# baowj-678/koordinator

Hardware: AMD Instinct MI355X
Metric: pods placed/sec + (pod,node) Filter+Score evals/sec at 50k nodes, 1-8 GPUs (higher is better)
Workload: dtype int64; 1 GPU; config4: 50000 nodes x 100000 pods, 30% BE, NodeResourcesFit + LoadAwareScheduling, shipped scheduler-config.yaml profile; nodes=50000, pods=100000, batch_pods=24, pipeline_lag=2, parallelism=node-shard x1

## Files before the change

koordinator_amd/csrc/eval.hpp:

```cpp
#pragma once
#include <hip/hip_runtime.h>
#include <stdint.h>

#include "../../include/koordhip.h"
#include "numa.hpp"

namespace kh {

template <typename T>
__device__ __forceinline__ void st_wt(T *p, T v) {
  if constexpr (sizeof(T) == 8) {
    __hip_atomic_store(reinterpret_cast<uint64_t *>(p), __builtin_bit_cast(uint64_t, v), __ATOMIC_RELAXED,
                       __HIP_MEMORY_SCOPE_AGENT);
  } else if constexpr (sizeof(T) == 4) {
    __hip_atomic_store(reinterpret_cast<uint32_t *>(p), __builtin_bit_cast(uint32_t, v), __ATOMIC_RELAXED,
                       __HIP_MEMORY_SCOPE_AGENT);
  } else {
    __hip_atomic_store(reinterpret_cast<uint8_t *>(p), __builtin_bit_cast(uint8_t, v), __ATOMIC_RELAXED,
                       __HIP_MEMORY_SCOPE_AGENT);
  }
}

enum : uint32_t {
  NF_LA_OK_NONPROD = 1u,
  NF_LA_OK_PROD = 2u,
  NF_LA_SCORE_ZERO = 4u,
  NF_OVER_CPU = 8u,
  NF_OVER_MEM = 16u,
  NF_OVER_EPH = 32u,
};

struct DevCfg {
  uint32_t filt, score;
  int32_t w_fit, w_la, w_numa, w_bal;
  int32_t fit_w[KOORDHIP_NRES];
  int32_t la_w_cpu, la_w_mem;
  int32_t according;
  int32_t la_alias;
  int32_t numa_w_cpu, numa_w_mem;
  int32_t numa_most;
  int32_t zones;
  int32_t amp;
  int32_t resv;
  int32_t resv_slots;
  int32_t resv_cpus;
  int32_t resv_b1;
  int32_t wide_keys;
  int32_t w_ext[KOORDHIP_NEXT_PLUGINS];
  int32_t dev_most;
  int32_t dev_w[5];
};

struct DevDev {
  int32_t slots;
  const uint8_t *present;
  const int32_t *minor;
  const int64_t *total;
  int64_t *used;
  const int64_t *xalloc;
  int64_t *xreq;
  const uint16_t *sscore[2];
  const int32_t *rslot;
  int64_t *rdev;
  const int64_t *rxa;
  int64_t *rxd;
};

struct DevNodes {
  const double *alloc[KOORDHIP_NRES];
  const int32_t *alloc_pods;
  double *requested[KOORDHIP_NRES];
  double *nz_cpu, *nz_mem;
// ... 68 lines not shown
  if (ns) {
    n.r_cpu |= !is_cpuset(p);
    n.r_mem = true;
    n.a_cpu = n.a_mem = true;
  }
  if (c.score & KOORDHIP_PLUGIN_BALANCED) n.r_cpu = n.r_mem = n.a_cpu = n.a_mem = true;
  n.sa = (c.filt & KOORDHIP_PLUGIN_NODE_STATIC) != 0;
  if (c.resv) {
    n.resv = true;
    n.r_cpu = n.r_mem = n.pods = true;
    n.eph |= (c.filt & KOORDHIP_PLUGIN_RESERVATION) && p.resv_match != 0ull;
  }
  n.a_cpu = n.a_cpu || n.r_cpu || n.nz_cpu || (n.la && c.la_alias);
  n.a_mem = n.a_mem || n.r_mem || n.nz_mem || (n.la && c.la_alias);
  return n;
}

__device__ __forceinline__ void need_or(Need &a, const Need &b) {
  a.pods |= b.pods;
  a.r_cpu |= b.r_cpu;
  a.r_mem |= b.r_mem;
  a.eph |= b.eph;
  a.bcpu |= b.bcpu;
  a.bmem |= b.bmem;
  a.a_cpu |= b.a_cpu;
  a.a_mem |= b.a_mem;
  a.nz_cpu |= b.nz_cpu;
  a.nz_mem |= b.nz_mem;
  a.la |= b.la;
  a.la_nonprod |= b.la_nonprod;
  a.la_prod |= b.la_prod;
  a.numa |= b.numa;
  a.numa_masks |= b.numa_masks;
  a.zones |= b.zones;
  a.amp |= b.amp;
  a.resv |= b.resv;
}

__device__ __forceinline__ Need need_all(const DevCfg &c) {
  Need n{};
  n.pods = n.r_cpu = n.r_mem = n.eph = n.bcpu = n.bmem = n.a_cpu = n.a_mem = n.nz_cpu = n.nz_mem = true;
  n.la = true;
  n.la_nonprod = true;
  n.la_prod = c.according != 0;
  n.numa = n.numa_masks = numa_on(c);
  n.zones = n.numa && c.zones;
  n.amp = n.numa && c.amp;
  n.resv = c.resv != 0;
  n.sa = true;
  return n;
}

__device__ __forceinline__ void load_zones(NumaRow &r, const DevNodes &d, int32_t i) {
  const double *zu = d.nu.zu + (size_t)i * 2 * ZMAX;
  r.za = d.nu.za + (size_t)i * 2 * ZMAX;
#pragma unroll
  for (int q = 0; q < ZMAX; q++) {
    r.zu[0][q] = zu[q];
    r.zu[1][q] = zu[ZMAX + q];
  }
}

template <bool Z>
__device__ __forceinline__ void load_numa(NumaRow &r, const DevNodes &d, int32_t i, const Need &n) {
  r.cls = -1;
  r.nflags = 0;
  r.amp = 1.0;
  if (!n.numa) return;
  r.cls = d.nu.node_cls[i];
  if (n.amp) {
    r.amp = d.nu.amp[i];
    r.cnt = d.nu.cnt[i];
  }
  if (n.numa_masks || (Z && n.zones)) r.nflags = d.nu.nflags[i];
  if constexpr (Z) {
    if (n.zones && topo_policy(r.nflags) != 0) load_zones(r, d, i);
  }
  if (n.numa_masks) {
    r.cnt = d.nu.cnt[i];
#pragma unroll
    for (int w = 0; w < NW; w++) {
      r.fr[w] = d.nu.fr[w][i];
      r.ep[w] = d.nu.ep[w][i];
      r.en[w] = d.nu.en[w][i];
    }
  }
}

template <typename T>
__device__ __forceinline__ const T &col(const T *base, int32_t i) {
  return *reinterpret_cast<const T *>(reinterpret_cast<const char *>(base) + (uint32_t)i * (uint32_t)sizeof(T));
}
template <typename T>
__device__ __forceinline__ T &col(T *base, int32_t i) {
  return *reinterpret_cast<T *>(reinterpret_cast<char *>(base) + (uint32_t)i * (uint32_t)sizeof(T));
}

__device__ __forceinline__ void load_node(NV &v, const DevNodes &d, int32_t i, const Need &n, const DevCfg &c) {
  v.flags = col(d.flags, i);
  v.sa = (n.sa && d.sallow) ? col(d.sallow, i) : 0xFFFFFFFFu;
  if (n.pods) {
    v.a_pods = col(d.alloc_pods, i);
    v.npods = col(d.npods, i);
  }
  if (n.a_cpu) v.a[KOORDHIP_RES_CPU] = col(d.alloc[KOORDHIP_RES_CPU], i);
  if (n.a_mem) v.a[KOORDHIP_RES_MEM] = col(d.alloc[KOORDHIP_RES_MEM], i);
  if (n.r_cpu) v.r[KOORDHIP_RES_CPU] = col(d.requested[KOORDHIP_RES_CPU], i);
// ... 266 lines not shown
    resv_pref_cpus(r, p, (c.score & KOORDHIP_PLUGIN_RESERVATION) ? mm : 0u, P, rx);
    NumaRow q = r;
    if (topo_policy(q.nflags) != 0) load_zones(q, *zd, zi);
    t = eval_total_numa<true>(p, w, q, classes, c, P);
  } else if constexpr (RC && S > 1) {
    uint64_t P[NW];
    resv_pref_cpus(r, p, (c.score & KOORDHIP_PLUGIN_RESERVATION) ? mm : 0u, P, rx);
    t = eval_total_numa<false>(p, w, r, classes, c, P);
  } else {
    t = eval_total_numa<false>(p, w, r, classes, c);
  }
  if (t < 0) return t;
  if (nmatch == 0)
    return ((c.filt & KOORDHIP_PLUGIN_RESERVATION) && (p.flags & KOORDHIP_POD_RESV_AFFINITY)) ? -1 : t;
  if ((c.filt & KOORDHIP_PLUGIN_RESERVATION) && !resv_filter(p, w, r, mm, nmatch, rx)) return -1;
  if (c.score & KOORDHIP_PLUGIN_RESERVATION) {
    const int rk = resv_node_rank(r, mm);
    if (rk >= 0) return 101 * c.resv_b1 + (KOORDHIP_RESV_MAX_ORDERS - 1 - rk);
    const int q = resv_nominate(p, r, mm, rx);
    if (q >= 0) t += resv_score(p, r.rs[q], q == rx.h, rx) * c.resv_b1;
  }
  return t;
}

__device__ __forceinline__ uint64_t make_key(int32_t total, int32_t node) {
  return total < 0 ? 0ull : (((uint64_t)(uint32_t)(total + 1)) << 32) | (uint64_t)(0xFFFFFFFFu - (uint32_t)node);
}
__device__ __forceinline__ int32_t key_node(uint64_t k) { return (int32_t)(0xFFFFFFFFu - (uint32_t)k); }
__device__ __forceinline__ int32_t key_score(uint64_t k) { return (int32_t)(k >> 32) - 1; }

__device__ __forceinline__ void apply_delta(NV &v, const DevPod &p, int sign) {
  const double sg = (double)sign;
#pragma unroll
  for (int r = 0; r < KOORDHIP_NRES; r++) v.r[r] = __builtin_fma(sg, p.req[r], v.r[r]);
  v.nz_cpu = __builtin_fma(sg, p.nz_cpu_m, v.nz_cpu);
  v.nz_mem = __builtin_fma(sg, p.nz_mem, v.nz_mem);
  v.npods += sign;
  v.la_u_cpu = __builtin_fma(sg, p.est_cpu, v.la_u_cpu);
  v.la_u_mem = __builtin_fma(sg, p.est_mem, v.la_u_mem);
  if (p.flags & KOORDHIP_POD_PROD) {
    v.la_up_cpu = __builtin_fma(sg, p.est_cpu, v.la_up_cpu);
    v.la_up_mem = __builtin_fma(sg, p.est_mem, v.la_up_mem);
  }
  uint32_t f = v.flags & ~(NF_OVER_CPU | NF_OVER_MEM | NF_OVER_EPH);
  if (v.r[KOORDHIP_RES_CPU] > v.a[KOORDHIP_RES_CPU]) f |= NF_OVER_CPU;
  if (v.r[KOORDHIP_RES_MEM] > v.a[KOORDHIP_RES_MEM]) f |= NF_OVER_MEM;
  if (v.r[KOORDHIP_RES_EPH] > v.a[KOORDHIP_RES_EPH]) f |= NF_OVER_EPH;
  v.flags = f;
}

__device__ __forceinline__ void load_row(NV &v, const DevNodes &d, int32_t i) {
#pragma unroll
  for (int r = 0; r < KOORDHIP_NRES; r++) {
    v.a[r] = d.alloc[r][i];
    v.r[r] = d.requested[r][i];
  }
  v.a_pods = d.alloc_pods[i];
  v.npods = d.npods[i];
  v.nz_cpu = d.nz_cpu[i];
  v.nz_mem = d.nz_mem[i];
  v.la_a_cpu = d.la_alloc_cpu[i];
  v.la_a_mem = d.la_alloc_mem[i];
  v.la_u_cpu = d.la_used_cpu[i];
  v.la_u_mem = d.la_used_mem[i];
  v.la_up_cpu = d.la_used_prod_cpu[i];
  v.la_up_mem = d.la_used_prod_mem[i];
  v.flags = d.flags[i];
  v.sa = d.sallow ? d.sallow[i] : 0xFFFFFFFFu;
}

template <bool Z = true>
__device__ __forceinline__ void load_numa_row(NumaRow &r, const DevNodes &d, int32_t i) {
  r.cls = d.nu.node_cls[i];
  r.nflags = d.nu.nflags[i];
  r.cnt = d.nu.cnt[i];
#pragma unroll
  for (int w = 0; w < NW; w++) {
    r.fr[w] = d.nu.fr[w][i];
    r.ep[w] = d.nu.ep[w][i];
    r.en[w] = d.nu.en[w][i];
  }
  if (Z && d.nu.za && topo_policy(r.nflags) != 0) load_zones(r, d, i);
  r.amp = d.nu.amp ? d.nu.amp[i] : 1.0;
}

template <bool Z = true>
__device__ __forceinline__ void store_numa_row(const NumaRow &r, const DevNodes &d, int32_t i) {
  d.nu.cnt[i] = r.cnt;
#pragma unroll
  for (int w = 0; w < NW; w++) {
    d.nu.fr[w][i] = r.fr[w];
    d.nu.ep[w][i] = r.ep[w];
    d.nu.en[w][i] = r.en[w];
  }
  if (Z && d.nu.za && topo_policy(r.nflags) != 0) {
    double *zu = d.nu.zu + (size_t)i * 2 * ZMAX;
#pragma unroll
    for (int q = 0; q < ZMAX; q++) {
      zu[q] = r.zu[0][q];
      zu[ZMAX + q] = r.zu[1][q];
    }
  }
}

__device__ __forceinline__ void numa_apply(NumaRow &r, const DevPod &p, const uint64_t *cpus, int sign,
                                           const uint64_t *P = nullptr) {
  const int ex = (int)KOORDHIP_NUMA_EXCLUSIVE(p.numa_policy);
  int n = 0;
#pragma unroll
  for (int w = 0; w < NW; w++) {
    n += __popcll(P ? (cpus[w] & ~P[w]) : cpus[w]);
    if (sign > 0) {
      r.fr[w] &= ~cpus[w];
      r.ep[w] = (r.ep[w] & ~cpus[w]) | (ex == (int)KOORDHIP_CPUEXCL_PCPU ? cpus[w] : 0ull);
      r.en[w] = (r.en[w] & ~cpus[w]) | (ex == (int)KOORDHIP_CPUEXCL_NUMA ? cpus[w] : 0ull);
    } else {
      r.fr[w] |= cpus[w];
      r.ep[w] &= ~cpus[w];
      r.en[w] &= ~cpus[w];
    }
  }
  r.cnt += sign * n;
}

__device__ __forceinline__ void store_row(const NV &v, const DevNodes &d, int32_t i) {
#pragma unroll
  for (int r = 0; r < KOORDHIP_NRES; r++) d.requested[r][i] = v.r[r];
  d.npods[i] = v.npods;
  d.nz_cpu[i] = v.nz_cpu;
  d.nz_mem[i] = v.nz_mem;
  d.la_used_cpu[i] = v.la_u_cpu;
  d.la_used_mem[i] = v.la_u_mem;
  d.la_used_prod_cpu[i] = v.la_up_cpu;
  d.la_used_prod_mem[i] = v.la_up_mem;
  d.flags[i] = (uint8_t)v.flags;
}

__device__ __forceinline__ void store_row_wt(const NV &v, const DevNodes &d, int32_t i) {
#pragma unroll
  for (int r = 0; r < KOORDHIP_NRES; r++) st_wt(&d.requested[r][i], v.r[r]);
  st_wt(&d.npods[i], v.npods);
  st_wt(&d.nz_cpu[i], v.nz_cpu);
  st_wt(&d.nz_mem[i], v.nz_mem);
  st_wt(&d.la_used_cpu[i], v.la_u_cpu);
  st_wt(&d.la_used_mem[i], v.la_u_mem);
  st_wt(&d.la_used_prod_cpu[i], v.la_up_cpu);
  st_wt(&d.la_used_prod_mem[i], v.la_up_mem);
  st_wt(&d.flags[i], (uint8_t)v.flags);
}

template <bool Z = true>
__device__ __forceinline__ void store_numa_row_wt(const NumaRow &r, const DevNodes &d, int32_t i) {
  st_wt(&d.nu.cnt[i], r.cnt);
#pragma unroll
  for (int w = 0; w < NW; w++) {
    st_wt(&d.nu.fr[w][i], r.fr[w]);
    st_wt(&d.nu.ep[w][i], r.ep[w]);
    st_wt(&d.nu.en[w][i], r.en[w]);
  }
  if (Z && d.nu.za && topo_policy(r.nflags) != 0) {
    double *zu = d.nu.zu + (size_t)i * 2 * ZMAX;
#pragma unroll
    for (int q = 0; q < ZMAX; q++) {
      st_wt(&zu[q], r.zu[0][q]);
      st_wt(&zu[ZMAX + q], r.zu[1][q]);
    }
  }
}

template <bool Z, bool WAVE = false>
__device__ __attribute__((noinline)) bool numa_reserve(const DevNumaClass *classes, NumaRow &row, const DevPod &pod,
                                                       uint64_t *cpus_out, const uint64_t *pref = nullptr) {
  NumaRow r = row;
  const DevPod p = pod;
  uint64_t cpus[NW] = {0, 0, 0, 0};
  uint64_t P[NW] = {0, 0, 0, 0};
  if (pref)
    for (int w = 0; w < NW; w++) P[w] = pref[w];
  for (int w = 0; w < NW; w++) cpus_out[w] = 0;
  const bool cs = (p.flags & KOORDHIP_POD_CPUSET) != 0;
  const int tp = Z ? topo_policy(r.nflags) : 0;
  if (!cs && tp == 0) return true;
  if (r.cls < 0) return false;
  const DevNumaClass &C = classes[r.cls];
  if (!Z || tp == 0) {
    if (cs && any4(P)) {
      if (!numa_allocate_pref_in<WAVE>(C, r, p, P, cpus)) return false;
    } else if (!numa_allocate_in<WAVE>(C, r, p, cpus)) {
      return false;
    }
    numa_apply(r, p, cpus, +1, P);
  } else {
    uint32_t mask;
    double av[2][ZMAX];
    zone_avail_all(r, C.nnuma, av);
    if (!zone_hint(C.nnuma, av, p, tp, &mask)) return false;
    const bool hp = cs && any4(P);
    if (hp) {
      double ru[ZMAX];
      zone_reusable(C, P, ru);
      zone_avail_reus(r, C.nnuma, ru, av);
    }
    double z[2][ZMAX];
    if (mask && !zone_alloc(C.nnuma, av, p, mask, z)) return false;
    if (cs) {
      if (mask) {
        if (!zone_allocate_in(C, r, p, z, cpus, hp ? P : nullptr)) return false;
      } else if (hp) {
        if (!numa_allocate_pref_in<WAVE>(C, r, p, P, cpus)) return false;
      } else if (!numa_allocate_in<WAVE>(C, r, p, cpus)) {
        return false;
      }
      numa_apply(r, p, cpus, +1, P);
    }
    if (mask) {
#pragma unroll
      for (int k = 0; k < ZMAX; k++) {
        r.zu[0][k] += z[0][k];
// ... 27 lines not shown
```

koordinator_amd/csrc/kernels.hip:

```cpp
#include <hip/hip_runtime.h>

#include <algorithm>
#include <cstdio>
#include <cstdlib>

#include "eval.hpp"
#include "karg.hpp"
#include "kernels.h"
#include "pipe.hpp"
#include "rows.hpp"

namespace kh {


__device__ __forceinline__ uint64_t shfl_u64(uint64_t v, int src) {
  uint32_t lo = __shfl((uint32_t)v, src, 64);
  uint32_t hi = __shfl((uint32_t)(v >> 32), src, 64);
  return ((uint64_t)hi << 32) | lo;
}
__device__ __forceinline__ uint64_t shfl_up_u64(uint64_t v, int d) {
  uint32_t lo = __shfl_up((uint32_t)v, d, 64);
  uint32_t hi = __shfl_up((uint32_t)(v >> 32), d, 64);
  return ((uint64_t)hi << 32) | lo;
}
// ... 1378 lines not shown
      if ((uint32_t)(kk >> 32) == S) st_wt(&o[mgt + pos++], kk);
    }
  }
  for (int32_t j = mgt + min(mneed, mties) + t; j < k; j += ETK_THREADS) st_wt(&o[j], (uint64_t)0);
  if (dbg && t == 0) {
    atomicAdd((unsigned long long *)&dbg[44], (unsigned long long)(stamp() - ts[3]));
    atomicAdd((unsigned long long *)&dbg[45], 1ull);
    atomicAdd((unsigned long long *)&dbg[46], (unsigned long long)total);
  }
  if (sy) {
    asm volatile("s_waitcnt vmcnt(0)" ::: "memory");
    __syncthreads();
    if (t == 0) pipe_count_pod(sy, sel_par);
  }
  }
  if (sy && res_wait > 0 && t == 0) (void)wait_at_least(&sy->res_round, res_wait, sy);
}


template <int NM>
constexpr int res_threads() { return NM ? 256 : 512; }
template <int NM>
constexpr int res_loaders() { return res_threads<NM>() >= 512 ? 3 : 1; }

constexpr int RES_PRE = 128;
constexpr int RES_HASH = 256;
constexpr int RES_WE = 8;
constexpr int RES_CHAIN_PASSES = 3;
constexpr int RES_LDS_MAX = 160 * 1024 - 3 * 1024;

constexpr int RES_WORDS = 20;
static_assert(sizeof(NV) == RES_WORDS * 8, "NV row = 20 words");
static_assert(offsetof(NV, r) == 40 && offsetof(NV, nz_cpu) == 80 && offsetof(NV, la_u_cpu) == 112 &&
                  offsetof(NV, la_up_cpu) == 128 && offsetof(NV, a_pods) == 144 && offsetof(NV, npods) == 148 &&
                  offsetof(NV, flags) == 152,
              "NV word layout");

__device__ __forceinline__ NV slot_row(const NV &src) {
  NV v = src;
  uint32_t f = v.flags & ~(uint32_t)(NF_OVER_CPU | NF_OVER_MEM | NF_OVER_EPH);
  if (v.r[KOORDHIP_RES_CPU] > v.a[KOORDHIP_RES_CPU]) f |= NF_OVER_CPU;
  if (v.r[KOORDHIP_RES_MEM] > v.a[KOORDHIP_RES_MEM]) f |= NF_OVER_MEM;
  if (v.r[KOORDHIP_RES_EPH] > v.a[KOORDHIP_RES_EPH]) f |= NF_OVER_EPH;
  v.flags = f;
  return v;
}

struct ResLds {
  int32_t dep;
  int32_t lists, pods, prev_rows, prev_numa, cur_rows, cur_numa, hash_node, hash_slot, pre_rows, pre_numa, pre_node,
      dec_key, dec_n, dec_src, dec_e, dec_c, moved, mhash, gbits, kpre, ktab, ready, classes, modmap, total;
  int32_t kwide;
  int32_t overlap, lists2, pods2, pre_rows2, pre_numa2, pre_node2;
};

__host__ __device__ inline int32_t res_align(int32_t x) { return (x + 15) & ~15; }

__host__ __device__ inline ResLds res_lds(int32_t n_pods_max, int32_t kp, int32_t n_nodes, int32_t nrow,
                                          bool overlap = false, bool tables = true, int32_t lag = 1,
                                          bool wide = false, bool chain = true) {
  const bool numa = nrow > 0;
  ResLds o;
  int32_t at = 0;
  const int32_t bitmap = res_align(((n_nodes + 31) >> 5) * 4);
  o.lists = at;
  at += res_align(n_pods_max * kp * 8);
  o.pods = at;
  at += res_align(n_pods_max * (int32_t)sizeof(DevPod));
  const int32_t rows_b = res_align(lag * n_pods_max * (int32_t)sizeof(NV));
  const int32_t numa_b = numa ? res_align(lag * n_pods_max * nrow) : 0;
  o.prev_rows = at;
  o.prev_numa = at + rows_b;
  at += rows_b + numa_b;
  o.cur_rows = at;
  o.cur_numa = at + rows_b;
  at += rows_b + numa_b;
  o.hash_node = at;
  at += RES_HASH * 4;
  o.hash_slot = at;
  at += RES_HASH * 4;
  o.pre_rows = at;
  at += res_align(RES_PRE * (int32_t)sizeof(NV));
  o.pre_numa = at;
  at += numa ? res_align(RES_PRE * nrow) : 0;
  o.pre_node = at;
  at += RES_PRE * 4;
  o.dec_key = at;
  at += RES_MAXP_ROUND * 8;
  o.dec_n = at;
  at += RES_MAXP_ROUND * 4;
  o.dec_src = at;
  at += RES_MAXP_ROUND * 4;
  o.dec_e = at;
  at += RES_MAXP_ROUND * RES_WE * 4;
  o.dec_c = at;
  at += RES_MAXP_ROUND * 4;
  o.dep = chain ? at : -1;
  at += chain ? RES_MAXP_ROUND * 8 : 0;
  o.moved = at;
  at += RES_MAXP_ROUND * 4;
  o.mhash = at;
  at += 2 * RES_MAXP_ROUND * 4;
  o.gbits = at;
  at += bitmap;
  o.kpre = o.ktab = -1;
  o.kwide = wide ? 1 : 0;
  o.ready = at;
  at += RES_MAXP_ROUND * 4;
  if (tables) {
    o.kpre = at;
    at += RES_MAXP_ROUND * RES_MAXP_ROUND * (wide ? 4 : 2);
    o.ktab = at;
    at += RES_MAXP_ROUND * RES_MAXP_ROUND * (wide ? 4 : 2);
  }
  o.classes = at;
  at += numa ? NUMA_LDS_CLASSES * (int32_t)sizeof(DevNumaClass) : 0;
  o.modmap = at;
  at += bitmap;
  o.overlap = overlap ? 1 : 0;
  o.lists2 = o.pods2 = o.pre_rows2 = o.pre_numa2 = o.pre_node2 = 0;
  if (overlap) {
    o.lists2 = at;
    at += res_align(n_pods_max * kp * 8);
    o.pods2 = at;
    at += res_align(n_pods_max * (int32_t)sizeof(DevPod));
    o.pre_rows2 = at;
    at += res_align(RES_PRE * (int32_t)sizeof(NV));
    o.pre_numa2 = at;
    at += numa ? res_align(RES_PRE * nrow) : 0;
    o.pre_node2 = at;
    at += RES_PRE * 4;
  }
  o.total = at;
  return o;
}

__device__ __forceinline__ uint32_t res_hash(int32_t node) { return ((uint32_t)node * 2654435761u) >> 24; }
__device__ __forceinline__ DevPod uniform_pod(const DevPod &src) {
  DevPod p;
  const uint32_t *s = reinterpret_cast<const uint32_t *>(&src);
  uint32_t *o = reinterpret_cast<uint32_t *>(&p);
#pragma unroll
  for (int i = 0; i < (int)(sizeof(DevPod) / 4); i++) o[i] = __builtin_amdgcn_readfirstlane(s[i]);
  return p;
}
__device__ __forceinline__ bool xbit(const uint32_t *m, int32_t nd) { return (m[nd >> 5] >> (nd & 31)) & 1u; }
__device__ __forceinline__ uint64_t ktab_key(uint32_t v, int32_t nd) {
  return v ? ((uint64_t)v << 32) | (uint64_t)(0xFFFFFFFFu - (uint32_t)nd) : 0ull;
}

__global__ void k_wait_resolved(PipeSync *sy, int32_t rounds) {
  if (threadIdx.x == 0) (void)wait_at_least(&sy->res_round, rounds, sy);
}
__global__ void k_signal_lists(PipeSync *sy, int32_t par, int32_t pods) {
  if (threadIdx.x == 0) store_release(&sy->sel[par], pods);
}

template <int NM, bool DBG>
__global__ __launch_bounds__(res_threads<NM>()) void k_resolve(DevCfg c, const DevNodes *__restrict__ dn, int32_t n_nodes,
                                                                 const DevNumaClass *__restrict__ ncls, const DevPod *__restrict__ pods,
                                                                 int32_t total, int32_t P, int32_t k, int32_t kp,
                                                                 int32_t r_begin, int32_t r_end,
                                                                 int32_t *__restrict__ mbuf,
                                                                 const uint64_t *__restrict__ lists0,
                                                                 int64_t list_buf, int32_t monotone, int32_t lag,
                                                                 PipeSync *sy, ResLds ofs, int32_t *__restrict__ out_node,
                                                                 uint64_t *__restrict__ out_cpus,
                                                                 uint64_t *__restrict__ dbg, int32_t trace) {
  constexpr int RES_THREADS = res_threads<NM>();
  constexpr bool NUMA = NM != 0, ZONES = NM == 2;
  if constexpr (!DBG) dbg = nullptr;
  using NR = side_row_t<NM>;
  (void)trace;
  extern __shared__ __attribute__((aligned(16))) char lds[];
  uint64_t *lk = reinterpret_cast<uint64_t *>(lds + ofs.lists);
  DevPod *lpod = reinterpret_cast<DevPod *>(lds + ofs.pods);
  NV *prow = reinterpret_cast<NV *>(lds + ofs.prev_rows);
  NR *pnr = reinterpret_cast<NR *>(lds + ofs.prev_numa);
  NV *mrow = reinterpret_cast<NV *>(lds + ofs.cur_rows);
  NR *mnr = reinterpret_cast<NR *>(lds + ofs.cur_numa);
  int32_t *hnode = reinterpret_cast<int32_t *>(lds + ofs.hash_node);
  int32_t *hslot = reinterpret_cast<int32_t *>(lds + ofs.hash_slot);
  NV *pre = reinterpret_cast<NV *>(lds + ofs.pre_rows);
  NR *prenr = reinterpret_cast<NR *>(lds + ofs.pre_numa);
  int32_t *pre_node = reinterpret_cast<int32_t *>(lds + ofs.pre_node);
  uint64_t *dec_key = reinterpret_cast<uint64_t *>(lds + ofs.dec_key);
  int32_t *dec_n = reinterpret_cast<int32_t *>(lds + ofs.dec_n);
  int32_t *dec_src = reinterpret_cast<int32_t *>(lds + ofs.dec_src);
  int32_t *dec_e = reinterpret_cast<int32_t *>(lds + ofs.dec_e);
  int32_t *dec_c = reinterpret_cast<int32_t *>(lds + ofs.dec_c);
  int32_t *moved = reinterpret_cast<int32_t *>(lds + ofs.moved);
  int32_t *seg_p = reinterpret_cast<int32_t *>(lds + ofs.mhash);
  uint32_t *gbits = reinterpret_cast<uint32_t *>(lds + ofs.gbits);
  char *kpre = lds + (ofs.kpre >= 0 ? ofs.kpre : 0);
  char *ktab = lds + (ofs.ktab >= 0 ? ofs.ktab : 0);
  const bool kwide = ofs.kwide != 0;
  auto kget = [kwide](const char *tb, int32_t x) -> uint32_t {
    return kwide ? reinterpret_cast<const uint32_t *>(tb)[x] : (uint32_t)reinterpret_cast<const uint16_t *>(tb)[x];
  };
  auto kput = [kwide](char *tb, int32_t x, uint32_t v) {
    if (kwide)
      reinterpret_cast<uint32_t *>(tb)[x] = v;
    else
      reinterpret_cast<uint16_t *>(tb)[x] = (uint16_t)v;
  };
  const bool have_tables = ofs.kpre >= 0;
  int32_t *ready = reinterpret_cast<int32_t *>(lds + ofs.ready);
  uint32_t *modmap = reinterpret_cast<uint32_t *>(lds + ofs.modmap);
  uint64_t *lk2 = reinterpret_cast<uint64_t *>(lds + ofs.lists2);
  DevPod *lpod2 = reinterpret_cast<DevPod *>(lds + ofs.pods2);
  NV *pre2 = reinterpret_cast<NV *>(lds + ofs.pre_rows2);
  NR *prenr2 = reinterpret_cast<NR *>(lds + ofs.pre_numa2);
  int32_t *pre_node2 = reinterpret_cast<int32_t *>(lds + ofs.pre_node2);
  __shared__ int32_t pnode[RES_MAXP_ROUND];
  __shared__ int32_t pgen[RES_MAXP_ROUND];
  __shared__ int32_t seg_w[RES_MAXP_ROUND];
  __shared__ int32_t ckey[RES_HASH], cval[RES_HASH];
  __shared__ int32_t sh_mp, sh_stop, sh_done, sh_chain;
  __shared__ uint64_t sh_rsv;
  const int t = threadIdx.x, lane = lane_id();
  const int32_t words = (n_nodes + 31) >> 5;
  const int32_t HP = max(1, RES_PRE / P);
  auto nodes = [dn]() -> DevNodes {
    const DevNodes *p = dn;
    asm volatile("" : "+s"(p));
    return *p;
  };
  const bool two = kp > 64;
  const bool chain_on = (monotone & 2) && ofs.dep >= 0;
  const uint64_t t_kernel = (dbg && t == 0) ? stamp() : 0;
  if (t == 0) {
    sh_mp = r_begin > 0 ? min(mbuf[0], P) : 0;
    sh_stop = 0;
  }
  for (int32_t x = t; x < words; x += RES_THREADS) {
    modmap[x] = 0;
    gbits[x] = 0;
  }
  for (int32_t x = t; x < RES_MAXP_ROUND; x += RES_THREADS) {
    moved[x] = 0;
    ready[x] = 0;
  }
  for (int32_t x = t; x < RES_HASH; x += RES_THREADS) {
    ckey[x] = -1;
    cval[x] = 64;
  }
  const DevNumaClass *cls = ncls;
  if constexpr (NUMA) {
    const int32_t nc = nodes().nu.ncls;
    if (nc <= NUMA_LDS_CLASSES) {
      uint4 *dst = reinterpret_cast<uint4 *>(lds + ofs.classes);
      const uint4 *src = reinterpret_cast<const uint4 *>(ncls);
      for (int32_t x = t; x < nc * (int32_t)(sizeof(DevNumaClass) / 16); x += RES_THREADS) dst[x] = src[x];
      cls = reinterpret_cast<const DevNumaClass *>(lds + ofs.classes);
    }
  }
  __syncthreads();
  if (t < sh_mp) {
    const int32_t nd = mbuf[1 + t];
    pnode[t] = nd;
    NV v;
    load_row(v, nodes(), nd);
    prow[t] = v;
    if constexpr (NUMA) {
      NR rr;
      load_side_row<NM>(rr, nodes(), nd);
      pnr[t] = rr;
    }
    atomicOr(&modmap[nd >> 5], 1u << (nd & 31));
  }
  __syncthreads();
  int32_t my_node = -1;
  auto word_doff = [](int q) -> int32_t {
    if (q >= 5 && q < 10) return (q - 5) * 8;
    if (q == 10 || q == 11) return (int32_t)offsetof(DevPod, nz_cpu_m) + (q - 10) * 8;
    if (q == 14 || q == 16) return (int32_t)offsetof(DevPod, est_cpu);
    if (q == 15 || q == 17) return (int32_t)offsetof(DevPod, est_mem);
    return -1;
  };
  const int32_t doff = word_doff(lane);
  uint64_t c_pro = 0, c_wait = 0, c_loop = 0, c_rel = 0, c_hash = 0, c_wb = 0;
  uint64_t c_w1wait = 0, c_w1load = 0, c_bar = 0;
  uint64_t c_l[4] = {0, 0, 0, 0};
  uint64_t n_slow = 0, n_miss = 0, n_staged = 0, n_bulk = 0, n_tab = 0;
  uint64_t c_g[2] = {0, 0};
  uint64_t c_nx[8] = {0, 0, 0, 0, 0, 0, 0, 0};
  uint64_t c_p[3] = {0, 0, 0}, n_p2 = 0, n_conf = 0, n_slowc = 0, n_void = 0;
  uint64_t c_cand = 0, n_evpass = 0, n_tready = 0;
  uint64_t c_gc[3] = {0, 0, 0}, n_ghit = 0;
  uint64_t c_chain = 0;
  uint64_t c_ch[4] = {0, 0, 0, 0};
  uint64_t c_rw[4] = {0, 0, 0, 0}, n_chbm = 0;
  uint64_t c_ext = 0, n_ext = 0;
  auto load_round = [&](int32_t rr, int32_t rp0, int32_t rn, uint64_t *Lk, DevPod *Lp, NV *Pr, NR *Pn,
                        int32_t *Pnode, int32_t tid, int32_t nth) {
    const uint64_t *L = lists0 + (size_t)(rr & (2 * lag - 1)) * list_buf;
    const int32_t tot = rn * k;
    int32_t nd[2];
#pragma unroll
    for (int u = 0; u < 2; u++) {
      const int32_t sl = tid + u * nth, j = sl / HP, q = sl - j * HP;
      nd[u] = -1;
      if (sl < RES_PRE && j < rn && q < k) {
        const uint64_t e = L[(size_t)j * k + q];
        if (e != 0) nd[u] = key_node(e);
      }
    }
    constexpr int LB = 4;
    const uint4 *L4 = reinterpret_cast<const uint4 *>(L);
    const int32_t n16 = (tot + 1) >> 1;
    auto put = [&](int32_t e, uint64_t v) {
      if (e < tot) {
        const int32_t j = e / k, q = e - j * k;
        Lk[j * kp + q] = v;
      }
    };
    uint4 lv[LB];
#pragma unroll
    for (int u = 0; u < LB; u++)
      if (tid + u * nth < n16) lv[u] = L4[tid + u * nth];
#pragma unroll
    for (int u = 0; u < LB; u++) {
      const int32_t x = tid + u * nth;
      if (x < n16) {
        put(2 * x, ((uint64_t)lv[u].y << 32) | lv[u].x);
        put(2 * x + 1, ((uint64_t)lv[u].w << 32) | lv[u].z);
      }
    }
    NV v[2];
#pragma unroll
    for (int u = 0; u < 2; u++)
      if (nd[u] >= 0) load_row(v[u], nodes(), nd[u]);
    for (int32_t x0 = tid + LB * nth; x0 < n16; x0 += LB * nth) {
#pragma unroll
      for (int u = 0; u < LB; u++)
        if (x0 + u * nth < n16) lv[u] = L4[x0 + u * nth];
#pragma unroll
      for (int u = 0; u < LB; u++) {
        const int32_t x = x0 + u * nth;
        if (x < n16) {
          put(2 * x, ((uint64_t)lv[u].y << 32) | lv[u].x);
          put(2 * x + 1, ((uint64_t)lv[u].w << 32) | lv[u].z);
        }
      }
    }
    for (int32_t x = tid; x < rn * (kp - k); x += nth) {
      const int32_t j = x / (kp - k), q = k + x - j * (kp - k);
      Lk[j * kp + q] = 0ull;
    }
    {
      const uint4 *src = reinterpret_cast<const uint4 *>(pods + rp0);
      uint4 *dst = reinterpret_cast<uint4 *>(Lp);
      const int32_t p16 = rn * (int32_t)(sizeof(DevPod) / 16);
      for (int32_t x0 = tid; x0 < p16; x0 += 4 * nth) {
        const int32_t x1 = x0 + nth, x2 = x0 + 2 * nth, x3 = x0 + 3 * nth;
        const uint4 a0 = src[x0];
        const uint4 a1 = x1 < p16 ? src[x1] : a0;
        const uint4 a2 = x2 < p16 ? src[x2] : a0;
        const uint4 a3 = x3 < p16 ? src[x3] : a0;
        dst[x0] = a0;
        if (x1 < p16) dst[x1] = a1;
        if (x2 < p16) dst[x2] = a2;
        if (x3 < p16) dst[x3] = a3;
      }
    }
#pragma unroll
    for (int u = 0; u < 2; u++) {
      const int32_t sl = tid + u * nth;
      if (sl >= RES_PRE) continue;
      if (nd[u] >= 0) {
        Pr[sl] = v[u];
        if constexpr (NUMA) {
          NR rr2;
          load_side_row<NM>(rr2, nodes(), nd[u]);
          Pn[sl] = rr2;
        }
      }
      Pnode[sl] = nd[u];
    }
    for (int32_t sl = tid + 2 * nth; sl < RES_PRE; sl += nth) {
      const int32_t j = sl / HP, q = sl - j * HP;
      int32_t n1 = -1;
      if (j < rn && q < k) {
        const uint64_t e = L[(size_t)j * k + q];
        if (e != 0) n1 = key_node(e);
      }
      if (n1 >= 0) {
        NV v1;
        load_row(v1, nodes(), n1);
        Pr[sl] = v1;
        if constexpr (NUMA) {
          NR rr2;
          load_side_row<NM>(rr2, nodes(), n1);
          Pn[sl] = rr2;
        }
      }
      Pnode[sl] = n1;
    }
  };
  auto prev_slot = [&](int32_t nd) -> int32_t {
    uint32_t h = res_hash(nd);
    for (;;) {
      const int32_t x = hnode[h];
      if (x == nd) return hslot[h];
      if (x < 0) return -1;
      h = (h + 1) & (RES_HASH - 1);
    }
  };
  for (int32_t r = r_begin, p0 = r_begin * P; r < r_end && p0 < total; r++, p0 += P) {
    const int32_t n_pods = min(P, total - p0);
    const bool preloaded = ofs.overlap && r > r_begin;
    const uint64_t t_w0 = (dbg && t == 0) ? stamp() : 0;
    if (!preloaded) {
      if (t == 0 && !wait_at_least(&sy->sel[r & 1], P * (r >> 1) + n_pods, sy)) sh_stop = 1;
      __syncthreads();
    }
    if (sh_stop) return;
// ... 1449 lines not shown
```

koordinator_amd/csrc/resv.hpp:

```cpp
#pragma once
#include <hip/hip_runtime.h>
#include <stdint.h>

#include "../../include/koordhip.h"

namespace kh {

struct ResvSlot {
  double ra[2], rd[2], rz[2];
  int32_t rn;
  uint32_t rf;
  int32_t rk;
  int32_t rdev;
};
static_assert(sizeof(ResvSlot) == 64, "reservation slot = 64 B");

template <int S, bool X = (S > KOORDHIP_RESV_SLOTS)>
struct NumaRowRS;
template <int S>
struct NumaRowRS<S, false> : NumaRow {
  static constexpr int kSlots = S;
  ResvSlot rs[S];
};
template <int S>
struct NumaRowRS<S, true> : NumaRow {
  static constexpr int kSlots = S;
  ResvSlot rs[S];
  uint64_t rcx[S - KOORDHIP_RESV_SLOTS][NW];
};
using NumaRowR = NumaRowRS<1>;
using NumaRowR4 = NumaRowRS<KOORDHIP_RESV_SLOTS>;
using NumaRowR8 = NumaRowRS<KOORDHIP_RESV_SLOTS_MAX>;

template <int S>
__device__ __forceinline__ uint64_t *rcm_of(NumaRowRS<S> &r, int q) {
  if constexpr (S > KOORDHIP_RESV_SLOTS) {
    return q < KOORDHIP_RESV_SLOTS ? r.rcm[q] : r.rcx[q - KOORDHIP_RESV_SLOTS];
  } else {
    return r.rcm[q];
  }
}
template <int S>
__device__ __forceinline__ const uint64_t *rcm_of(const NumaRowRS<S> &r, int q) {
  if constexpr (S > KOORDHIP_RESV_SLOTS) {
    return q < KOORDHIP_RESV_SLOTS ? r.rcm[q] : r.rcx[q - KOORDHIP_RESV_SLOTS];
  } else {
    return r.rcm[q];
  }
}

constexpr double RESV_NZ_CPU = 100.0;
constexpr double RESV_NZ_MEM = 200.0 * 1024.0 * 1024.0;

template <int S>
__device__ __forceinline__ void load_resv(NumaRowRS<S> &r, const DevResv &d, int32_t i) {
#pragma unroll
  for (int q = 0; q < S; q++) {
    ResvSlot &x = r.rs[q];
    const size_t at = (size_t)q * (size_t)d.stride + (size_t)i;
    x.rf = q < d.slots ? d.flags[at] : 0u;
    x.rn = 0;
    x.rk = 0;
    x.rdev = 0;
#pragma unroll
    for (int k = 0; k < 2; k++) x.ra[k] = x.rd[k] = x.rz[k] = 0.0;
    if (x.rf & KOORDHIP_RESV_PRESENT) {
      x.rn = d.rn[at];
      x.rk = d.rank[at];
#pragma unroll
      for (int k = 0; k < 2; k++) {
        x.ra[k] = d.ra[k][at];
        x.rd[k] = d.rd[k][at];
        x.rz[k] = d.rz[k][at];
      }
    }
    if constexpr (S > 1) {
      const bool on = d.rc[0] != nullptr && (x.rf & KOORDHIP_RESV_PRESENT);
#pragma unroll
      for (int w = 0; w < NW; w++) rcm_of(r, q)[w] = on ? d.rc[w][at] : 0ull;
    }
  }
}

template <int S>
__device__ __forceinline__ void store_resv(const NumaRowRS<S> &r, const DevResv &d, int32_t i) {
#pragma unroll
  for (int q = 0; q < S; q++) {
    const ResvSlot &x = r.rs[q];
    if (!(x.rf & KOORDHIP_RESV_PRESENT)) continue;
    const size_t at = (size_t)q * (size_t)d.stride + (size_t)i;
    d.rd[0][at] = x.rd[0];
    d.rd[1][at] = x.rd[1];
    d.rn[at] = x.rn;
    if constexpr (S > 1) {
      if (d.rc[0])
#pragma unroll
        for (int w = 0; w < NW; w++) d.rc[w][at] = rcm_of(r, q)[w];
    }
  }
}
template <int S>
__device__ __forceinline__ void store_resv_wt(const NumaRowRS<S> &r, const DevResv &d, int32_t i) {
#pragma unroll
  for (int q = 0; q < S; q++) {
    const ResvSlot &x = r.rs[q];
    if (!(x.rf & KOORDHIP_RESV_PRESENT)) continue;
    const size_t at = (size_t)q * (size_t)d.stride + (size_t)i;
    st_wt(&d.rd[0][at], x.rd[0]);
    st_wt(&d.rd[1][at], x.rd[1]);
    st_wt(&d.rn[at], x.rn);
    if constexpr (S > 1) {
      if (d.rc[0])
#pragma unroll
        for (int w = 0; w < NW; w++) st_wt(&d.rc[w][at], rcm_of(r, q)[w]);
    }
  }
}

__device__ __forceinline__ bool rkey(uint32_t rf, int k) {
  return (rf & (k == 0 ? KOORDHIP_RESV_KEY_CPU : KOORDHIP_RESV_KEY_MEM)) != 0;
}
__device__ __forceinline__ bool pkey(const DevPod &p, int k) {
  return (p.flags & (k == 0 ? KOORDHIP_POD_KEY_CPU : KOORDHIP_POD_KEY_MEM)) != 0;
}
__device__ __forceinline__ double rem_of(const ResvSlot &r, int k) {
  const double x = r.ra[k] - r.rd[k];
  return rkey(r.rf, k) && x > 0.0 ? x : 0.0;
}

enum : uint32_t { RX_REM = 1u, RX_FIT_H = 2u, RX_FIT_O = 4u, RX_LE = 8u, RX_INTER = 16u, RX_NZ = 32u, RX_XFIT = 64u };
struct ResvXS {
  int32_t h;
  uint32_t f;
  int32_t xs, xw;
};
__device__ __forceinline__ ResvXS no_rx() { return ResvXS{-1, 0u, 0, 0}; }

__device__ __forceinline__ int resv_class(const ResvSlot &r, const DevPod &p) {
  if (!(r.rf & KOORDHIP_RESV_PRESENT)) return 0;
  if ((r.rf & KOORDHIP_RESV_ALLOCATE_ONCE) && r.rn > 0) return 0;
  const bool match = (p.resv_match >> KOORDHIP_RESV_GROUP(r.rf)) & 1ull;
  if (!(r.rf & KOORDHIP_RESV_UNSCHEDULABLE) && match) return 1;
  return r.rn > 0 ? 2 : 0;
}

template <int S>
__device__ __forceinline__ int resv_restore(NV &v, const NumaRowRS<S> &r, const DevPod &p, uint32_t &mm,
                                            ResvXS rx = no_rx()) {
  int nmatch = 0;
  bool touched = false;
  mm = 0;
#pragma unroll
  for (int q = 0; q < S; q++) {
    const ResvSlot &x = r.rs[q];
    const int cls = resv_class(x, p);
    if (cls == 0) continue;
    touched = true;
    v.r[KOORDHIP_RES_CPU] -= x.ra[0];
    v.r[KOORDHIP_RES_MEM] -= x.ra[1];
    v.nz_cpu -= x.rz[0];
    v.nz_mem -= x.rz[1];
    if (cls == 1) {
      v.npods -= 1;
      nmatch++;
      mm |= 1u << q;
    } else {
      const double rc = rem_of(x, 0), rm = rem_of(x, 1);
// ... 194 lines not shown
```

Measured before the change: 1.694 million pods/s.

## Use global address-space loads/stores, cache node pointer table in LDS, prefetch row staging

Casts node-row and reservation loads and write-through stores to address_space(1), so the compiler emits global rather than flat memory instructions. For small NM the DevNodes pointer table is copied into LDS once per block, replacing repeated scalar loads from the device struct. The list/pod staging routine is reworked: list entries, pod data and the first node rows are issued up front, and the list copy loop is software-pipelined with a deeper unroll (4 to 6) using clamped indices. This aims to cut flat-address overhead and pointer-chasing latency, at the cost of extra LDS, more registers and redundant clamped loads.

```diff
diff --git a/koordinator_amd/csrc/eval.hpp b/koordinator_amd/csrc/eval.hpp
--- a/koordinator_amd/csrc/eval.hpp
+++ b/koordinator_amd/csrc/eval.hpp
@@ -18,6 +18,23 @@
   } else {
     __hip_atomic_store(reinterpret_cast<uint8_t *>(p), __builtin_bit_cast(uint8_t, v), __ATOMIC_RELAXED,
                        __HIP_MEMORY_SCOPE_AGENT);
+  }
+}
+
+template <typename T>
+using gptr = __attribute__((address_space(1))) T *;
+template <typename T>
+__device__ __forceinline__ gptr<T> as_global(T *p) {
+  return (gptr<T>)p;
+}
+template <typename T>
+__device__ __forceinline__ void st_wt_g(T *p, T v) {
+  if constexpr (sizeof(T) == 8) {
+    __hip_atomic_store((gptr<uint64_t>)p, __builtin_bit_cast(uint64_t, v), __ATOMIC_RELAXED, __HIP_MEMORY_SCOPE_AGENT);
+  } else if constexpr (sizeof(T) == 4) {
+    __hip_atomic_store((gptr<uint32_t>)p, __builtin_bit_cast(uint32_t, v), __ATOMIC_RELAXED, __HIP_MEMORY_SCOPE_AGENT);
+  } else {
+    __hip_atomic_store((gptr<uint8_t>)p, __builtin_bit_cast(uint8_t, v), __ATOMIC_RELAXED, __HIP_MEMORY_SCOPE_AGENT);
   }
 }
 
@@ -192,7 +209,7 @@
 }
 
 __device__ __forceinline__ void load_zones(NumaRow &r, const DevNodes &d, int32_t i) {
-  const double *zu = d.nu.zu + (size_t)i * 2 * ZMAX;
+  const gptr<const double> zu = as_global<const double>(d.nu.zu) + (size_t)i * 2 * ZMAX;
   r.za = d.nu.za + (size_t)i * 2 * ZMAX;
 #pragma unroll
   for (int q = 0; q < ZMAX; q++) {
@@ -565,36 +582,36 @@
 __device__ __forceinline__ void load_row(NV &v, const DevNodes &d, int32_t i) {
 #pragma unroll
   for (int r = 0; r < KOORDHIP_NRES; r++) {
-    v.a[r] = d.alloc[r][i];
-    v.r[r] = d.requested[r][i];
-  }
-  v.a_pods = d.alloc_pods[i];
-  v.npods = d.npods[i];
-  v.nz_cpu = d.nz_cpu[i];
-  v.nz_mem = d.nz_mem[i];
-  v.la_a_cpu = d.la_alloc_cpu[i];
-  v.la_a_mem = d.la_alloc_mem[i];
-  v.la_u_cpu = d.la_used_cpu[i];
-  v.la_u_mem = d.la_used_mem[i];
-  v.la_up_cpu = d.la_used_prod_cpu[i];
-  v.la_up_mem = d.la_used_prod_mem[i];
-  v.flags = d.flags[i];
-  v.sa = d.sallow ? d.sallow[i] : 0xFFFFFFFFu;
+    v.a[r] = as_global(d.alloc[r])[i];
+    v.r[r] = as_global(d.requested[r])[i];
+  }
+  v.a_pods = as_global(d.alloc_pods)[i];
+  v.npods = as_global(d.npods)[i];
+  v.nz_cpu = as_global(d.nz_cpu)[i];
+  v.nz_mem = as_global(d.nz_mem)[i];
+  v.la_a_cpu = as_global(d.la_alloc_cpu)[i];
+  v.la_a_mem = as_global(d.la_alloc_mem)[i];
+  v.la_u_cpu = as_global(d.la_used_cpu)[i];
+  v.la_u_mem = as_global(d.la_used_mem)[i];
+  v.la_up_cpu = as_global(d.la_used_prod_cpu)[i];
+  v.la_up_mem = as_global(d.la_used_prod_mem)[i];
+  v.flags = as_global(d.flags)[i];
+  v.sa = d.sallow ? as_global(d.sallow)[i] : 0xFFFFFFFFu;
 }
 
 template <bool Z = true>
 __device__ __forceinline__ void load_numa_row(NumaRow &r, const DevNodes &d, int32_t i) {
-  r.cls = d.nu.node_cls[i];
-  r.nflags = d.nu.nflags[i];
-  r.cnt = d.nu.cnt[i];
+  r.cls = as_global(d.nu.node_cls)[i];
+  r.nflags = as_global(d.nu.nflags)[i];
+  r.cnt = as_global(d.nu.cnt)[i];
 #pragma unroll
   for (int w = 0; w < NW; w++) {
-    r.fr[w] = d.nu.fr[w][i];
-    r.ep[w] = d.nu.ep[w][i];
-    r.en[w] = d.nu.en[w][i];
+    r.fr[w] = as_global(d.nu.fr[w])[i];
+    r.ep[w] = as_global(d.nu.ep[w])[i];
+    r.en[w] = as_global(d.nu.en[w])[i];
   }
   if (Z && d.nu.za && topo_policy(r.nflags) != 0) load_zones(r, d, i);
-  r.amp = d.nu.amp ? d.nu.amp[i] : 1.0;
+  r.amp = d.nu.amp ? as_global(d.nu.amp)[i] : 1.0;
 }
 
 template <bool Z = true>
@@ -651,32 +668,32 @@
 
 __device__ __forceinline__ void store_row_wt(const NV &v, const DevNodes &d, int32_t i) {
 #pragma unroll
-  for (int r = 0; r < KOORDHIP_NRES; r++) st_wt(&d.requested[r][i], v.r[r]);
-  st_wt(&d.npods[i], v.npods);
-  st_wt(&d.nz_cpu[i], v.nz_cpu);
-  st_wt(&d.nz_mem[i], v.nz_mem);
-  st_wt(&d.la_used_cpu[i], v.la_u_cpu);
-  st_wt(&d.la_used_mem[i], v.la_u_mem);
-  st_wt(&d.la_used_prod_cpu[i], v.la_up_cpu);
-  st_wt(&d.la_used_prod_mem[i], v.la_up_mem);
-  st_wt(&d.flags[i], (uint8_t)v.flags);
+  for (int r = 0; r < KOORDHIP_NRES; r++) st_wt_g(&d.requested[r][i], v.r[r]);
+  st_wt_g(&d.npods[i], v.npods);
+  st_wt_g(&d.nz_cpu[i], v.nz_cpu);
+  st_wt_g(&d.nz_mem[i], v.nz_mem);
+  st_wt_g(&d.la_used_cpu[i], v.la_u_cpu);
+  st_wt_g(&d.la_used_mem[i], v.la_u_mem);
+  st_wt_g(&d.la_used_prod_cpu[i], v.la_up_cpu);
+  st_wt_g(&d.la_used_prod_mem[i], v.la_up_mem);
+  st_wt_g(&d.flags[i], (uint8_t)v.flags);
 }
 
 template <bool Z = true>
 __device__ __forceinline__ void store_numa_row_wt(const NumaRow &r, const DevNodes &d, int32_t i) {
-  st_wt(&d.nu.cnt[i], r.cnt);
+  st_wt_g(&d.nu.cnt[i], r.cnt);
 #pragma unroll
   for (int w = 0; w < NW; w++) {
-    st_wt(&d.nu.fr[w][i], r.fr[w]);
-    st_wt(&d.nu.ep[w][i], r.ep[w]);
-    st_wt(&d.nu.en[w][i], r.en[w]);
+    st_wt_g(&d.nu.fr[w][i], r.fr[w]);
+    st_wt_g(&d.nu.ep[w][i], r.ep[w]);
+    st_wt_g(&d.nu.en[w][i], r.en[w]);
   }
   if (Z && d.nu.za && topo_policy(r.nflags) != 0) {
     double *zu = d.nu.zu + (size_t)i * 2 * ZMAX;
 #pragma unroll
     for (int q = 0; q < ZMAX; q++) {
-      st_wt(&zu[q], r.zu[0][q]);
-      st_wt(&zu[ZMAX + q], r.zu[1][q]);
+      st_wt_g(&zu[q], r.zu[0][q]);
+      st_wt_g(&zu[ZMAX + q], r.zu[1][q]);
     }
   }
 }
diff --git a/koordinator_amd/csrc/kernels.hip b/koordinator_amd/csrc/kernels.hip
--- a/koordinator_amd/csrc/kernels.hip
+++ b/koordinator_amd/csrc/kernels.hip
@@ -1454,9 +1454,15 @@
       dec_key, dec_n, dec_src, dec_e, dec_c, moved, mhash, gbits, kpre, ktab, ready, classes, modmap, total;
   int32_t kwide;
   int32_t overlap, lists2, pods2, pre_rows2, pre_numa2, pre_node2;
+  int32_t ptab;
 };
 
 __host__ __device__ inline int32_t res_align(int32_t x) { return (x + 15) & ~15; }
+
+__host__ __device__ inline int32_t res_ptab_bytes(int32_t nrow) {
+  if (nrow == 0) return res_align((int32_t)offsetof(DevNodes, nu));
+  return nrow == (int32_t)sizeof(NumaRow) ? res_align((int32_t)offsetof(DevNodes, rv)) : 0;
+}
 
 __host__ __device__ inline ResLds res_lds(int32_t n_pods_max, int32_t kp, int32_t n_nodes, int32_t nrow,
                                           bool overlap = false, bool tables = true, int32_t lag = 1,
@@ -1519,6 +1525,8 @@
   at += numa ? NUMA_LDS_CLASSES * (int32_t)sizeof(DevNumaClass) : 0;
   o.modmap = at;
   at += bitmap;
+  o.ptab = res_ptab_bytes(nrow) ? at : -1;
+  at += res_ptab_bytes(nrow);
   o.overlap = overlap ? 1 : 0;
   o.lists2 = o.pods2 = o.pre_rows2 = o.pre_numa2 = o.pre_node2 = 0;
   if (overlap) {
@@ -1623,11 +1631,20 @@
   const int t = threadIdx.x, lane = lane_id();
   const int32_t words = (n_nodes + 31) >> 5;
   const int32_t HP = max(1, RES_PRE / P);
-  auto nodes = [dn]() -> DevNodes {
-    const DevNodes *p = dn;
-    asm volatile("" : "+s"(p));
-    return *p;
+  auto nodes = [&]() -> decltype(auto) {
+    if constexpr (NM <= 2) {
+      return *reinterpret_cast<const DevNodes *>(lds + ofs.ptab);
+    } else {
+      const DevNodes *p = dn;
+      asm volatile("" : "+s"(p));
+      return DevNodes(*p);
+    }
   };
+  if constexpr (NM <= 2) {
+    constexpr int PW = (int)((NUMA ? offsetof(DevNodes, rv) : offsetof(DevNodes, nu)) / 8);
+    static_assert(PW <= RES_THREADS, "one 8-byte word of the pointer table per thread");
+    if (t < PW) reinterpret_cast<uint64_t *>(lds + ofs.ptab)[t] = reinterpret_cast<const uint64_t *>(dn)[t];
+  }
   const bool two = kp > 64;
   const bool chain_on = (monotone & 2) && ofs.dep >= 0;
   const uint64_t t_kernel = (dbg && t == 0) ? stamp() : 0;
@@ -1649,7 +1666,7 @@
   }
   const DevNumaClass *cls = ncls;
   if constexpr (NUMA) {
-    const int32_t nc = nodes().nu.ncls;
+    const int32_t nc = dn->nu.ncls;
     if (nc <= NUMA_LDS_CLASSES) {
       uint4 *dst = reinterpret_cast<uint4 *>(lds + ofs.classes);
       const uint4 *src = reinterpret_cast<const uint4 *>(ncls);
@@ -1698,17 +1715,15 @@
                         int32_t *Pnode, int32_t tid, int32_t nth) {
     const uint64_t *L = lists0 + (size_t)(rr & (2 * lag - 1)) * list_buf;
     const int32_t tot = rn * k;
-    int32_t nd[2];
+    uint64_t he[2] = {0, 0};
+    bool hv[2];
 #pragma unroll
     for (int u = 0; u < 2; u++) {
       const int32_t sl = tid + u * nth, j = sl / HP, q = sl - j * HP;
-      nd[u] = -1;
-      if (sl < RES_PRE && j < rn && q < k) {
-        const uint64_t e = L[(size_t)j * k + q];
-        if (e != 0) nd[u] = key_node(e);
-      }
-    }
-    constexpr int LB = 4;
+      hv[u] = sl < RES_PRE && j < rn && q < k;
+      if (u * nth < RES_PRE) he[u] = L[min(j * k + q, tot - 1)];
+    }
+    constexpr int LB = 6;
     const uint4 *L4 = reinterpret_cast<const uint4 *>(L);
     const int32_t n16 = (tot + 1) >> 1;
     auto put = [&](int32_t e, uint64_t v) {
@@ -1717,54 +1732,64 @@
         Lk[j * kp + q] = v;
       }
     };
+    auto put2 = [&](int32_t x, const uint4 &w) {
+      if (x < n16) {
+        put(2 * x, ((uint64_t)w.y << 32) | w.x);
+        put(2 * x + 1, ((uint64_t)w.w << 32) | w.z);
+      }
+    };
     uint4 lv[LB];
 #pragma unroll
     for (int u = 0; u < LB; u++)
-      if (tid + u * nth < n16) lv[u] = L4[tid + u * nth];
-#pragma unroll
-    for (int u = 0; u < LB; u++) {
-      const int32_t x = tid + u * nth;
-      if (x < n16) {
-        put(2 * x, ((uint64_t)lv[u].y << 32) | lv[u].x);
-        put(2 * x + 1, ((uint64_t)lv[u].w << 32) | lv[u].z);
-      }
-    }
+      if (u * nth < n16) lv[u] = L4[min(tid + u * nth, n16 - 1)];
+    const uint4 *psrc = reinterpret_cast<const uint4 *>(pods + rp0);
+    uint4 *pdst = reinterpret_cast<uint4 *>(Lp);
+    const int32_t p16 = rn * (int32_t)(sizeof(DevPod) / 16);
+    uint4 a0, a1, a2, a3;
+    a0 = psrc[min(tid, p16 - 1)];
+    if (nth < p16) a1 = psrc[min(tid + nth, p16 - 1)];
+    if (2 * nth < p16) a2 = psrc[min(tid + 2 * nth, p16 - 1)];
+    if (3 * nth < p16) a3 = psrc[min(tid + 3 * nth, p16 - 1)];
+    int32_t nd[2];
     NV v[2];
 #pragma unroll
-    for (int u = 0; u < 2; u++)
-      if (nd[u] >= 0) load_row(v[u], nodes(), nd[u]);
-    for (int32_t x0 = tid + LB * nth; x0 < n16; x0 += LB * nth) {
-#pragma unroll
-      for (int u = 0; u < LB; u++)
-        if (x0 + u * nth < n16) lv[u] = L4[x0 + u * nth];
-#pragma unroll
-      for (int u = 0; u < LB; u++) {
-        const int32_t x = x0 + u * nth;
-        if (x < n16) {
-          put(2 * x, ((uint64_t)lv[u].y << 32) | lv[u].x);
-          put(2 * x + 1, ((uint64_t)lv[u].w << 32) | lv[u].z);
-        }
-      }
+    for (int u = 0; u < 2; u++) {
+      nd[u] = (hv[u] && he[u] != 0) ? key_node(he[u]) : -1;
+      if (u * nth < RES_PRE)
+        if (nd[u] >= 0) load_row(v[u], nodes(), nd[u]);
+    }
+    for (int32_t b = 0;;) {
+      const int32_t nb = b + LB * nth;
+      const bool more = nb < n16;
+      uint4 nx[LB];
+      if (more) {
+#pragma unroll
+        for (int u = 0; u < LB; u++)
+          if (nb + u * nth < n16) nx[u] = L4[min(nb + tid + u * nth, n16 - 1)];
+      }
+#pragma unroll
+      for (int u = 0; u < LB; u++) put2(b + tid + u * nth, lv[u]);
+      if (!more) break;
+#pragma unroll
+      for (int u = 0; u < LB; u++) lv[u] = nx[u];
+      b = nb;
     }
     for (int32_t x = tid; x < rn * (kp - k); x += nth) {
       const int32_t j = x / (kp - k), q = k + x - j * (kp - k);
       Lk[j * kp + q] = 0ull;
     }
-    {
-      const uint4 *src = reinterpret_cast<const uint4 *>(pods + rp0);
-      uint4 *dst = reinterpret_cast<uint4 *>(Lp);
-      const int32_t p16 = rn * (int32_t)(sizeof(DevPod) / 16);
-      for (int32_t x0 = tid; x0 < p16; x0 += 4 * nth) {
-        const int32_t x1 = x0 + nth, x2 = x0 + 2 * nth, x3 = x0 + 3 * nth;
-        const uint4 a0 = src[x0];
-        const uint4 a1 = x1 < p16 ? src[x1] : a0;
-        const uint4 a2 = x2 < p16 ? src[x2] : a0;
-        const uint4 a3 = x3 < p16 ? src[x3] : a0;
-        dst[x0] = a0;
-        if (x1 < p16) dst[x1] = a1;
-        if (x2 < p16) dst[x2] = a2;
-        if (x3 < p16) dst[x3] = a3;
-      }
+    if (tid < p16) pdst[tid] = a0;
+    if (tid + nth < p16) pdst[tid + nth] = a1;
+    if (tid + 2 * nth < p16) pdst[tid + 2 * nth] = a2;
+    if (tid + 3 * nth < p16) pdst[tid + 3 * nth] = a3;
+    for (int32_t b = 4 * nth; b < p16; b += 4 * nth) {
+      const int32_t x0 = b + tid, x1 = x0 + nth, x2 = x0 + 2 * nth, x3 = x0 + 3 * nth;
+      const uint4 c0 = psrc[min(x0, p16 - 1)], c1 = psrc[min(x1, p16 - 1)], c2 = psrc[min(x2, p16 - 1)],
+                  c3 = psrc[min(x3, p16 - 1)];
+      if (x0 < p16) pdst[x0] = c0;
+      if (x1 < p16) pdst[x1] = c1;
+      if (x2 < p16) pdst[x2] = c2;
+      if (x3 < p16) pdst[x3] = c3;
     }
 #pragma unroll
     for (int u = 0; u < 2; u++) {
diff --git a/koordinator_amd/csrc/resv.hpp b/koordinator_amd/csrc/resv.hpp
--- a/koordinator_amd/csrc/resv.hpp
+++ b/koordinator_amd/csrc/resv.hpp
@@ -58,26 +58,26 @@
   for (int q = 0; q < S; q++) {
     ResvSlot &x = r.rs[q];
     const size_t at = (size_t)q * (size_t)d.stride + (size_t)i;
-    x.rf = q < d.slots ? d.flags[at] : 0u;
+    x.rf = q < d.slots ? as_global(d.flags)[at] : 0u;
     x.rn = 0;
     x.rk = 0;
     x.rdev = 0;
 #pragma unroll
     for (int k = 0; k < 2; k++) x.ra[k] = x.rd[k] = x.rz[k] = 0.0;
     if (x.rf & KOORDHIP_RESV_PRESENT) {
-      x.rn = d.rn[at];
-      x.rk = d.rank[at];
+      x.rn = as_global(d.rn)[at];
+      x.rk = as_global(d.rank)[at];
 #pragma unroll
       for (int k = 0; k < 2; k++) {
-        x.ra[k] = d.ra[k][at];
-        x.rd[k] = d.rd[k][at];
-        x.rz[k] = d.rz[k][at];
+        x.ra[k] = as_global(d.ra[k])[at];
+        x.rd[k] = as_global(d.rd[k])[at];
+        x.rz[k] = as_global(d.rz[k])[at];
       }
     }
     if constexpr (S > 1) {
       const bool on = d.rc[0] != nullptr && (x.rf & KOORDHIP_RESV_PRESENT);
 #pragma unroll
-      for (int w = 0; w < NW; w++) rcm_of(r, q)[w] = on ? d.rc[w][at] : 0ull;
+      for (int w = 0; w < NW; w++) rcm_of(r, q)[w] = on ? as_global(d.rc[w])[at] : 0ull;
     }
   }
 }
@@ -106,13 +106,13 @@
     const ResvSlot &x = r.rs[q];
     if (!(x.rf & KOORDHIP_RESV_PRESENT)) continue;
     const size_t at = (size_t)q * (size_t)d.stride + (size_t)i;
-    st_wt(&d.rd[0][at], x.rd[0]);
-    st_wt(&d.rd[1][at], x.rd[1]);
-    st_wt(&d.rn[at], x.rn);
+    st_wt_g(&d.rd[0][at], x.rd[0]);
+    st_wt_g(&d.rd[1][at], x.rd[1]);
+    st_wt_g(&d.rn[at], x.rn);
     if constexpr (S > 1) {
       if (d.rc[0])
 #pragma unroll
-        for (int w = 0; w < NW; w++) st_wt(&d.rc[w][at], rcm_of(r, q)[w]);
+        for (int w = 0; w < NW; w++) st_wt_g(&d.rc[w][at], rcm_of(r, q)[w]);
     }
   }
 }
```

After: 1.737 million pods/s (median of 6 runs). 2.6% higher.
